# 011235813/discrete_mean_field_game

Hardware: AMD Instinct MI355X
Metric: env-steps/sec for batched d-bin population rollouts (higher is better)
Workload: dtype f32 (f64 accumulate); 1 GPU; actor_critic.train(update_every="rollout") of the drop-in class (mfg_ac2.train call surface; device-side start draw every episode, one update per 15-step rollout): d=21 topics, T=15, global batch 65536 = 65536 trajectories per GPU x 1; d=21, T=15, batch_per_gpu=65536, global_batch=65536, rng=philox4x32-10, parallelism=trajectory-sharded x1, 1 all-reduce/update

## Files before the change

### discrete_mean_field_game_amd/csrc/mfg_batch_sums.hip

```cpp
#include <hip/hip_runtime.h>
#include <limits.h>
#include <stdint.h>

#include "../../include/mfg_hip.h"
#include "mfg_batch_sums.h"
#include "mfg_core.h"
#include "mfg_grad.h"
#include "mfg_host.h"
#include "mfg_population.h"

using namespace mfg;

__global__ __launch_bounds__(BLOCK) void k_grad_partial(GradArgs a) { grad_partial_body(a); }

__global__ void k_add_reward(double* __restrict__ delta, const float* __restrict__ reward, int64_t N) {
  for (int64_t n = blockIdx.x * (int64_t)blockDim.x + threadIdx.x; n < N; n += (int64_t)gridDim.x * blockDim.x)
    delta[n] += (double)reward[n];
}

__global__ __launch_bounds__(RP_SLICES* RP_OUT) void k_reduce_partials(const double* __restrict__ partial, int64_t nsb, int64_t FO,
                                                                      int accumulate, double* __restrict__ G, ReduceApply ap) { reduce_partials_body(partial, nsb, FO, accumulate, G, ap); }

constexpr unsigned GM2_RECT44 = 0xFFFFu, GM2_DIAG44 = 0x8CEFu, GM2_DIAG44M = 0x0CEFu, GM2_TRAP24 = 0xEFu, GM2_RECT24 = 0xFFu,
                   GM2_ONE = 1u;
__host__ __device__ constexpr int gm2_count(unsigned m) { return m == 0 ? 0 : (int)(m & 1u) + gm2_count(m >> 1); }

template <int D, int NA, int NB, unsigned MASK>
__device__ __forceinline__ void gm2_step(const float* __restrict__ abase, const float* __restrict__ bbase, int off, double dk,
                                         v4d_t* acc) {
  double av[NA], bv[NB];
#pragma unroll
  for (int i = 0; i < NA; ++i) av[i] = dk * (double)abase[off + (i << 4)];
#pragma unroll
  for (int j = 0; j < NB; ++j) bv[j] = (double)bbase[off + (j << 4)];
  int t = 0;
#pragma unroll
  for (int i = 0; i < NA; ++i) {
#pragma unroll
    for (int j = 0; j < NB; ++j) {
      if ((MASK >> (i * NB + j)) & 1u) {
        acc[t] = __builtin_amdgcn_mfma_f64_16x16x4f64(av[i], bv[j], acc[t], 0, 0, 0);
        ++t;
      }
    }
  }
}
template <int D, int NA0, int NB0, unsigned M0, int NA1, int NB1, unsigned M1>
__device__ __forceinline__ void gm2_chunk(const float* __restrict__ sp, const double* __restrict__ dl, int lk, int li,
                                          const int* ra, const int* cb, v4d_t* acc) {
  constexpr int pitch = D + 16;
  const float* lb = sp + lk * pitch + li;
  const float *a0 = lb + (ra[0] << 4), *b0 = lb + (cb[0] << 4), *a1 = lb + (ra[1] << 4), *b1 = lb + (cb[1] << 4);
#pragma unroll 2
  for (int ks = 0; ks < GM_KC / 4; ++ks) {
    const double dk = dl[ks * 4 + lk];
    gm2_step<D, NA0, NB0, M0>(a0, b0, ks * 4 * pitch, dk, acc);
    if constexpr (M1 != 0) gm2_step<D, NA1, NB1, M1>(a1, b1, ks * 4 * pitch, dk, acc + gm2_count(M0));
  }
}
template <int D, int NA, int NB, unsigned MASK>
__device__ __forceinline__ void gm2_store(double* __restrict__ out, int lk, int li, int ra, int cb, const v4d_t* acc) {
  int t = 0;
#pragma unroll
  for (int i = 0; i < NA; ++i) {
#pragma unroll
    for (int j = 0; j < NB; ++j) {
      if ((MASK >> (i * NB + j)) & 1u) {
#pragma unroll
        for (int v = 0; v < 4; ++v) {
          const int gi = ((ra + i) << 4) + 4 * v + lk, gj = ((cb + j) << 4) + li;
          if (gi <= gj) out[feat_idx(gi, gj, D)] = acc[t][v];
        }
        ++t;
      }
    }
  }
}

template <int D>
struct Gm2Geom {
  static constexpr int NY = D == 256 ? 2 : 1, ACCN = D == 256 ? 17 : 9;
};
template <int NA_, int NB_, unsigned MASK_>
struct Gm2Rect {
  static constexpr int NA = NA_, NB = NB_;
  static constexpr unsigned MASK = MASK_;
};
template <int D>
__global__ __launch_bounds__(BLOCK, 2) void k_grad_mfma2(GradArgs a) {
  static_assert(D == 128 || D == 256, "tile maps exist for d = 128 and 256");
  extern __shared__ __attribute__((aligned(16))) unsigned char smem_raw[];
  constexpr int d = D, pitch = D + 16;
  constexpr int Q = d * (d + 1) / 2, F = Q + d + 1, FO = F + 3;
  constexpr int ACCN = Gm2Geom<D>::ACCN;
  double* dl = reinterpret_cast<double*>(smem_raw);
  double* red = dl + GM_KC;
  float* sp = reinterpret_cast<float*>(red + 4 * BLOCK);
  const int tid = threadIdx.x, lane = tid & (WAVE - 1);
  const int wv = __builtin_amdgcn_readfirstlane(tid / WAVE), y = (int)blockIdx.y;
  const bool diag = D == 256 ? wv == 3 : wv >= 2;
  int ra[2] = {0, 0}, cb[2] = {0, 0};
  if (D == 256) {
    const int sd = 2 * y;
    if (diag) {
      ra[0] = cb[0] = 4 * sd;
      ra[1] = cb[1] = 4 * sd + 4;
    } else {
      const int sr = y == 0 ? 0 : (wv == 2 ? 2 : 1), sc = y == 0 ? wv + 1 : (wv == 0 ? 2 : 3);
      ra[0] = 4 * sr;
      cb[0] = 4 * sc;
      ra[1] = 4 * sd + 4 + (wv == 2 ? 3 : 2);
      cb[1] = 4 * sd + 4 + (wv == 0 ? 2 : 3);
    }
  } else {
    if (diag) ra[0] = cb[0] = 4 * (wv - 2);
    else {
      ra[0] = 2 * wv;
      cb[0] = 4;
      ra[1] = cb[1] = 4 * wv + 3;
    }
  }
  const bool side = blockIdx.y == 0;
  double lin = 0.0, s_d = 0.0, s_dg = 0.0, s_r = 0.0, s_n = 0.0;
  const int li = lane & 15, lk = lane >> 4;
  const double invT = 1.0 / (double)a.T;
  constexpr int dq = d >> 2, rpp = BLOCK / dq, NPF = GM_KC / rpp;
  static_assert(BLOCK % dq == 0 && GM_KC % rpp == 0, "whole rows per staging pass");
  const int q0 = tid / dq, c4 = tid - q0 * dq;
  double* out = a.partial + (int64_t)blockIdx.x * FO;
  auto run = [&](auto r0, auto r1) __attribute__((always_inline)) {
    using R0 = decltype(r0);
    using R1 = decltype(r1);
    v4d_t acc[ACCN];
#pragma unroll
    for (int i = 0; i < ACCN; ++i) acc[i] = (v4d_t)(0.0);
    float4 pf[NPF];
    double pf_de = 0.0, pf_dg = 0.0, pf_rr = 0.0;
    bool pf_on = false;
    auto fetch = [&](int64_t n0_) __attribute__((always_inline)) {
      const int cn_ = (int)((a.N - n0_) < GM_KC ? (a.N - n0_) : GM_KC);
#pragma unroll
      for (int u = 0; u < NPF; ++u) {
        const int q = q0 + u * rpp;
        pf[u] = make_float4(0.f, 0.f, 0.f, 0.f);
        if (q < cn_) {
          const int64_t n = n0_ + q;
          const int64_t b = (int64_t)(((double)n + 0.5) * invT);
          pf[u] = *reinterpret_cast<const float4*>(a.pi + b * a.stride_b + (n - b * a.T) * d + 4 * c4);
        }
      }
      pf_de = 0.0, pf_dg = 0.0, pf_rr = 0.0, pf_on = false;
      if (tid < cn_) {
        const int64_t n = n0_ + tid;
        pf_de = a.delta[n];
        pf_rr = a.reward ? (double)a.reward[n] : 0.0;
// ... 145 lines not shown
  const double invT = 1.0 / (double)TP1;
  const int64_t npass = (N + VM2_MB - 1) / VM2_MB;
  const int ur = tid >> 2, uc = (tid & 3) << 4;
  const int xr = tid >> 4, xc = (tid & 15) << 2;
  double ustg[16];
  float4 xstg[8];
  for (int64_t pass = blockIdx.x; pass < npass; pass += gridDim.x) {
    const int64_t n0 = pass * VM2_MB;
    const float* xrow[8];
#pragma unroll
    for (int u = 0; u < 8; ++u) {
      int64_t n = n0 + xr + 16 * u;
      if (n >= N) n = N - 1;
      const int64_t b = (int64_t)(((double)n + 0.5) * invT);
      xrow[u] = pi + b * stride_b + (n - b * TP1) * (int64_t)d;
    }
    auto fetch = [&](int cbk, int kc) __attribute__((always_inline)) {
      const int k = VM2_KC * kc + ur, c0 = 64 * cbk + uc;
      const double* wr = w + ((int64_t)k * d - ((int64_t)k * (k - 1)) / 2 - k);
#pragma unroll
      for (int q = 0; q < 16; ++q) ustg[q] = (c0 + q >= k) ? wr[c0 + q] : 0.0;
#pragma unroll
      for (int u = 0; u < 8; ++u) xstg[u] = *reinterpret_cast<const float4*>(xrow[u] + VM2_KC * kc + xc);
    };
    auto commit = [&]() __attribute__((always_inline)) {
#pragma unroll
      for (int q = 0; q < 16; q += 2) *reinterpret_cast<double2*>(Us + ur * 64 + uc + q) = make_double2(ustg[q], ustg[q + 1]);
#pragma unroll
      for (int u = 0; u < 8; ++u) {
        float* dst = Xs + (xr + 16 * u) * VM2_XP + xc;
        *reinterpret_cast<float2*>(dst) = make_float2(xstg[u].x, xstg[u].y);
        *reinterpret_cast<float2*>(dst + 2) = make_float2(xstg[u].z, xstg[u].w);
      }
    };
    double vs[2][4] = {{0.0, 0.0, 0.0, 0.0}, {0.0, 0.0, 0.0, 0.0}};
    fetch(0, 0);
    for (int cbk = 0; cbk < ncb; ++cbk) {
      v4d_t acc[2][4];
#pragma unroll
      for (int sg = 0; sg < 2; ++sg)
#pragma unroll
        for (int cg = 0; cg < 4; ++cg) acc[sg][cg] = (v4d_t)(0.0);
      for (int kc = 0; kc <= cbk; ++kc) {
        __syncthreads();
        commit();
        __syncthreads();
        const bool last_kc = kc == cbk;
        if (!last_kc || cbk + 1 < ncb) fetch(last_kc ? cbk + 1 : cbk, last_kc ? 0 : kc + 1);
        const float* xa = Xs + (wv * 32 + li) * VM2_XP + lk;
        const double* ub = Us + lk * 64 + li;
        if (!last_kc) {
#pragma unroll 2
          for (int ks = 0; ks < VM2_KC / 4; ++ks) {
            const double a0 = (double)xa[4 * ks], a1 = (double)xa[16 * VM2_XP + 4 * ks];
#pragma unroll
            for (int cg = 0; cg < 4; ++cg) {
              const double bv = ub[4 * ks * 64 + 16 * cg];
              acc[0][cg] = __builtin_amdgcn_mfma_f64_16x16x4f64(a0, bv, acc[0][cg], 0, 0, 0);
              acc[1][cg] = __builtin_amdgcn_mfma_f64_16x16x4f64(a1, bv, acc[1][cg], 0, 0, 0);
            }
          }
        } else {
#pragma unroll
          for (int pq = 0; pq < 4; ++pq) {
#pragma unroll 2
            for (int ks = 4 * pq; ks < 4 * pq + 4; ++ks) {
              const double a0 = (double)xa[4 * ks], a1 = (double)xa[16 * VM2_XP + 4 * ks];
#pragma unroll
              for (int cg = pq; cg < 4; ++cg) {
                const double bv = ub[4 * ks * 64 + 16 * cg];
                acc[0][cg] = __builtin_amdgcn_mfma_f64_16x16x4f64(a0, bv, acc[0][cg], 0, 0, 0);
                acc[1][cg] = __builtin_amdgcn_mfma_f64_16x16x4f64(a1, bv, acc[1][cg], 0, 0, 0);
              }
            }
          }
        }
      }
#pragma unroll
      for (int cg = 0; cg < 4; ++cg) {
        const double bc = w[Q + 64 * cbk + 16 * cg + li];
#pragma unroll
        for (int sg = 0; sg < 2; ++sg) {
#pragma unroll
          for (int v = 0; v < 4; ++v) {
            const double x = (double)Xs[(wv * 32 + sg * 16 + 4 * v + lk) * VM2_XP + 16 * cg + li];
            vs[sg][v] = fma(acc[sg][cg][v] + bc, x, vs[sg][v]);
          }
        }
      }
    }
#pragma unroll
    for (int sg = 0; sg < 2; ++sg) {
#pragma unroll
      for (int v = 0; v < 4; ++v) {
        double t = vs[sg][v];
        t += dpp_mov_f64<0xB1, 0xF>(t);
        t += dpp_mov_f64<0x4E, 0xF>(t);
        t += dpp_mov_f64<0x141, 0xF>(t);
        t += dpp_mov_f64<0x140, 0xF>(t);
        const int64_t n = n0 + wv * 32 + sg * 16 + 4 * v + lk;
        if (li == 0 && n < N) V[n] = t + w[Q + d];
      }
    }
  }
}

__global__ void k_td_delta(const double* __restrict__ V, const float* __restrict__ reward, int64_t B, int T, double gamma,
                           int discount_pow, double* __restrict__ delta) {
  const int64_t n_tot = B * T;
  for (int64_t n = blockIdx.x * (int64_t)blockDim.x + threadIdx.x; n < n_tot; n += (int64_t)gridDim.x * blockDim.x) {
    const int64_t b = n / T;
    const int s = (int)(n - b * T);
    double gd = gamma;
    if (discount_pow) {
      gd = 1.0;
      for (int q = 0; q < s; ++q) gd *= gamma;
    }
    const double r = reward ? (double)reward[n] : 0.0;
    delta[n] = r + gd * V[b * (T + 1) + s + 1] - V[b * (T + 1) + s];
  }
}


namespace mfg {

bool value_batch_ok(int d) { return d > WAVE && d % 16 == 0 && d <= MFG_MAX_D; }
size_t value_buffer_bytes(int64_t N, int d) { return value_batch_ok(d) ? (size_t)(2 * N) * 8 : 0; }

void grad_geometry(int64_t N, int d, int* chunk, int64_t* nsb, int* nob) {
  const int64_t FO = mfg_num_features(d) + 3;
  int ch = 8192 / d;
  if (ch > 64) ch = 64;
  if (ch < 8) ch = 8;
  *chunk = ch;
  int64_t sb = (N + ch - 1) / ch;
#ifndef MFG_GRAD_WS_MB
#define MFG_GRAD_WS_MB 72
#endif
  int64_t cap = (int64_t)((long long)MFG_GRAD_WS_MB << 20) / (FO * 8);
  if (cap > 1024) cap = 1024;
  if (cap < 16) cap = 16;
  if (sb > cap) sb = cap;
  if (sb < 1) sb = 1;
  *nsb = sb;
  *nob = (int)((FO + GR_OUT_PER_BLOCK - 1) / GR_OUT_PER_BLOCK);
}

void launch_reduce_partials(const double* partial, int64_t nsb, int64_t FO, int accumulate, double* G, const ReduceApply& ap,
                            hipStream_t st) {
  hipLaunchKernelGGL(k_reduce_partials, dim3((unsigned)((FO + RP_OUT - 1) / RP_OUT)), dim3(RP_SLICES * RP_OUT), 0, st, partial, nsb,
                     FO, accumulate, G, ap);
}

int launch_grad(const float* pi, int64_t stride_b, const double* delta, const double* g, const float* reward, int64_t N, int T,
                int d, double* G, int accumulate, void* ws, size_t ws_bytes, hipStream_t st, const ApplyArgs* apply, bool* applied,
                bool add_reward, const PopArgs* pop) {
  if (applied) *applied = false;
  if (d <= MFG_GRAD_SMALL_MAX_D && T > INT_MAX - GS_CH)
    return fail(MFG_EUNSUPPORTED, "batch sums, d <= %d: T = %d above 2^31 - 65", MFG_GRAD_SMALL_MAX_D, T);
  const int64_t FO = mfg_num_features(d) + 3;
  int chunk, nob;
  int64_t nsb;
  grad_geometry(N, d, &chunk, &nsb, &nob);
  const size_t need = (size_t)(nsb * FO * 8) + MFG_WS_CONTROL_BYTES;
  if (ws_bytes < need) return fail(MFG_EWORKSPACE, "%s: need %lld bytes, have %lld", "workspace", (long long)need,
                                   (long long)ws_bytes);
  ReduceApply rap{};
  if (apply && !accumulate) {
    rap.on = 1;
    rap.lr_c = apply->lr_c;
    rap.lr_a = apply->lr_a;
    rap.count = (double)N;
    rap.w = apply->w;
    rap.theta = apply->theta;
    rap.reward_acc = apply->reward_acc;
  }
  GradArgs a{};
  a.pi = pi;
  a.stride_b = stride_b;
  a.delta = delta;
  a.g = g;
  a.reward = reward;
  a.N = N;
  a.T = T;
  a.d = d;
  a.chunk = chunk;
  a.nsb = nsb;
  a.partial = reinterpret_cast<double*>((char*)ws + MFG_WS_CONTROL_BYTES);
  const bool small = d <= MFG_GRAD_SMALL_MAX_D;
  if (add_reward && !small)
    hipLaunchKernelGGL(k_add_reward, dim3(grid_for(N, 256, 8)), dim3(256), 0, st, const_cast<double*>(delta), reward, N);
  if (small) {
    a.add_reward = add_reward ? 1 : 0;
    const int64_t NC = (N + GS_CH - 1) / GS_CH;
    int64_t blocks = (NC + WAVES - 1) / WAVES;
    const int64_t cap = (int64_t)num_cus() * MFG_GS_BPC;
    if (blocks > cap) blocks = cap;
    if (blocks > nsb) blocks = nsb;
    if (blocks < 1) blocks = 1;
    a.nsb = blocks;
    const bool fuse = blocks <= MFG_GRAD_FUSE_MAX_ROWS;
    if (fuse) {
      a.counter = reinterpret_cast<unsigned*>(ws);
      a.G = G;
      a.accumulate = accumulate;
      if (apply) {
        a.apply = 1;
        a.lr_c = apply->lr_c;
        a.lr_a = apply->lr_a;
        a.w = apply->w;
        a.theta = apply->theta;
        a.reward_acc = apply->reward_acc;
        if (applied) *applied = true;
      }
    }
    const bool wide = stride_b - (int64_t)T * d >= (1 << 23) || T >= MFG_GRAD_LONG_T;
    if (pop) {
      if (wide) return fail(MFG_EUNSUPPORTED, "%s", "population: trajectory stride or length beyond the small gradient kernel");
      launch_grad_mfma_small_pop(d == 21 || d == 15 ? d : 0, (unsigned)blocks, a, *pop, st);
      if (fuse) return check_launch("grad_mfma_small_pop");
      launch_reduce_partials_pop((unsigned)((FO + RP_OUT - 1) / RP_OUT), (const double*)a.partial, blocks, FO, G, rap, *pop, st);
      if (applied && rap.on) *applied = true;
      return check_launch("grad_mfma_small_pop");
    }
    if (wide) hipLaunchKernelGGL((k_grad_mfma_small<0, true>), dim3((unsigned)blocks), dim3(BLOCK), 0, st, a);
    else if (d == 21) hipLaunchKernelGGL((k_grad_mfma_small<21>), dim3((unsigned)blocks), dim3(BLOCK), 0, st, a);
    else if (d == 15) hipLaunchKernelGGL((k_grad_mfma_small<15>), dim3((unsigned)blocks), dim3(BLOCK), 0, st, a);
    else hipLaunchKernelGGL((k_grad_mfma_small<0>), dim3((unsigned)blocks), dim3(BLOCK), 0, st, a);
    if (fuse) return check_launch("grad_mfma_small");
    launch_reduce_partials(a.partial, blocks, FO, accumulate, G, rap, st);
    if (applied && rap.on) *applied = true;
    return check_launch("grad_mfma_small");
  }
  if (d % 16 == 0 && d >= 64 && d <= 4 * BLOCK) {
    const int nt = d / 16, ntiles = nt * (nt + 1) / 2;
    const int ny = (ntiles + WAVES * GM_TPW - 1) / (WAVES * GM_TPW);
    const int tpw = (ntiles + ny * WAVES - 1) / (ny * WAVES);
    a.chunk = (BLOCK % (d / 4) == 0 && (((uintptr_t)pi & 15) == 0) && (stride_b % 4 == 0)) ? 1 : 0;
    const size_t lds_m = (size_t)GM_KC * 8 + (size_t)4 * BLOCK * 8 + (size_t)GM_KC * (d + 16) * 4;
    const int npf = a.chunk ? d / 32 : 0;
    if (pop) {
      if (npf != 0 && npf != 2) return fail(MFG_EUNSUPPORTED, "%s", "population: d > 64");
      launch_grad_mfma_pop(npf, (unsigned)nsb, (unsigned)ny, lds_m, a, tpw, *pop, st);
      launch_reduce_partials_pop((unsigned)((FO + RP_OUT - 1) / RP_OUT), (const double*)a.partial, nsb, FO, G, rap, *pop, st);
      if (applied && rap.on) *applied = true;
      return check_launch("grad_mfma_pop");
    }
#ifndef MFG_GRAD_MFMA_OLD
    if (a.chunk && (d == 128 || d == 256)) {
#ifndef MFG_GM2_BPC128
#define MFG_GM2_BPC128 3
#endif
      const int64_t want = d == 256 ? (int64_t)num_cus() * 2 / Gm2Geom<256>::NY : (int64_t)num_cus() * MFG_GM2_BPC128 / Gm2Geom<128>::NY;
      if (nsb > want) nsb = want;
      a.nsb = nsb;
      if (d == 256) hipLaunchKernelGGL((k_grad_mfma2<256>), dim3((unsigned)nsb, (unsigned)Gm2Geom<256>::NY), dim3(BLOCK), lds_m, st, a);
      else hipLaunchKernelGGL((k_grad_mfma2<128>), dim3((unsigned)nsb, (unsigned)Gm2Geom<128>::NY), dim3(BLOCK), lds_m, st, a);
    } else
#endif
    switch (npf) {
      case 2: hipLaunchKernelGGL((k_grad_mfma<2>), dim3((unsigned)nsb, (unsigned)ny), dim3(BLOCK), lds_m, st, a, tpw); break;
      case 4: hipLaunchKernelGGL((k_grad_mfma<4>), dim3((unsigned)nsb, (unsigned)ny), dim3(BLOCK), lds_m, st, a, tpw); break;
      case 8: hipLaunchKernelGGL((k_grad_mfma<8>), dim3((unsigned)nsb, (unsigned)ny), dim3(BLOCK), lds_m, st, a, tpw); break;
      case 16: hipLaunchKernelGGL((k_grad_mfma<16>), dim3((unsigned)nsb, (unsigned)ny), dim3(BLOCK), lds_m, st, a, tpw); break;
      default: hipLaunchKernelGGL((k_grad_mfma<0>), dim3((unsigned)nsb, (unsigned)ny), dim3(BLOCK), lds_m, st, a, tpw); break;
    }
    launch_reduce_partials(a.partial, nsb, FO, accumulate, G, rap, st);
    if (applied && rap.on) *applied = true;
    return check_launch("grad_mfma");
  }
  const size_t lds = (size_t)chunk * 3 * 8 + (size_t)chunk * d * 4;
  if (pop) {
    launch_grad_partial_pop((unsigned)nsb, (unsigned)nob, lds, a, *pop, st);
    launch_reduce_partials_pop((unsigned)((FO + RP_OUT - 1) / RP_OUT), (const double*)a.partial, nsb, FO, G, rap, *pop, st);
    if (applied && rap.on) *applied = true;
    return check_launch("grad_partial_pop");
  }
  hipLaunchKernelGGL(k_grad_partial, dim3((unsigned)nsb, (unsigned)nob), dim3(BLOCK), lds, st, a);
  launch_reduce_partials(a.partial, nsb, FO, accumulate, G, rap, st);
  if (applied && rap.on) *applied = true;
  return check_launch("grad_reduce");
}

int launch_values_and_delta(const float* pi_traj, int64_t B, int T, int d, const double* w, const float* reward,
                                   double gamma, int discount_pow, double* delta, void* ws, size_t ws_bytes, hipStream_t st) {
  const int64_t N = B * T, NV = B * (int64_t)(T + 1);
  int chunk, nob;
  int64_t nsb;
  grad_geometry(N, d, &chunk, &nsb, &nob);
  const size_t off = (size_t)(nsb * (mfg_num_features(d) + 3) * 8) + MFG_WS_CONTROL_BYTES;
  if (!ws || ws_bytes < off + (size_t)NV * 8)
    return fail(MFG_EWORKSPACE, "%s: need %lld bytes, have %lld", "values", (long long)(off + (size_t)NV * 8), (long long)ws_bytes);
  double* V = reinterpret_cast<double*>((char*)ws + off);
  const size_t lds = (size_t)WAVES * 16 * (d + 4) * 4 + (size_t)2 * VM_CH * 16 * 8;
  int64_t groups = (NV + 15) / 16;
  int64_t blocks = (groups + WAVES - 1) / WAVES;
  const int64_t cap = (int64_t)num_cus() * 8;
  if (blocks > cap) blocks = cap;
#ifndef MFG_VALUE_MFMA_OLD
  if (d % 64 == 0) {
    const size_t lds2 = (size_t)VM2_KC * 64 * 8 + (size_t)VM2_MB * VM2_XP * 4;
    int64_t blocks2 = (NV + VM2_MB - 1) / VM2_MB;
    if (blocks2 > (int64_t)num_cus() * 2) blocks2 = (int64_t)num_cus() * 2;
    hipLaunchKernelGGL(k_value_mfma2, dim3((unsigned)blocks2), dim3(BLOCK), lds2, st, pi_traj, (int64_t)(T + 1) * d, NV, T + 1, d, w, V);
  } else
#endif
  hipLaunchKernelGGL(k_value_mfma, dim3((unsigned)blocks), dim3(BLOCK), lds, st, pi_traj, (int64_t)(T + 1) * d, NV, T + 1, d, w, V);
  hipLaunchKernelGGL(k_td_delta, dim3(grid_for(N, 256, 8)), dim3(256), 0, st, (const double*)V, reward, B, T, gamma, discount_pow,
                     delta);
  return check_launch("values");
}

}
```

### discrete_mean_field_game_amd/csrc/mfg_grad.h

```cpp
#pragma once
#include <hip/hip_runtime.h>
#include <stdint.h>

#include "mfg_core.h"

using namespace mfg;

constexpr int MFG_GRAD_SMALL_MAX_D = 28;
constexpr int GR_OUT_PER_THREAD = 4;
constexpr int GR_OUT_PER_BLOCK = GR_OUT_PER_THREAD * BLOCK;

struct GradArgs {
  const float* pi;
  int64_t stride_b;
  const double* delta;
  const double* g;
  const float* reward;
  int64_t N;
  int T, d, chunk;
  int64_t nsb;
  double* partial;
  int add_reward;
  unsigned* counter;
  double* G;
  int accumulate, apply;
  double lr_c, lr_a;
  double *w, *theta, *reward_acc;
};

__device__ __forceinline__ void grad_partial_body(const GradArgs& a) {
  extern __shared__ __attribute__((aligned(16))) unsigned char smem_raw[];
  const int d = a.d, Q = d * (d + 1) / 2, F = Q + d + 1, FO = F + 3;
  double* dl = reinterpret_cast<double*>(smem_raw);
  float* sp = reinterpret_cast<float*>(dl + 3 * a.chunk);
  const int tid = threadIdx.x;
  int oi[GR_OUT_PER_THREAD], oj[GR_OUT_PER_THREAD], kind[GR_OUT_PER_THREAD];
  double acc[GR_OUT_PER_THREAD];
#pragma unroll
  for (int u = 0; u < GR_OUT_PER_THREAD; ++u) {
    const int k = blockIdx.y * GR_OUT_PER_BLOCK + u * BLOCK + tid;
    acc[u] = 0.0;
    oi[u] = oj[u] = 0;
    if (k < Q) {
      int i = (int)(((2.0 * d + 1.0) - sqrt((2.0 * d + 1.0) * (2.0 * d + 1.0) - 8.0 * (double)k)) * 0.5);
      while (i > 0 && feat_idx(i, i, d) > k) --i;
      while (i + 1 < d && feat_idx(i + 1, i + 1, d) <= k) ++i;
      oi[u] = i;
      oj[u] = i + (k - feat_idx(i, i, d));
      kind[u] = 0;
    } else if (k < Q + d) {
      oi[u] = k - Q;
      kind[u] = 1;
    } else if (k < FO) {
      kind[u] = 2 + (k - (Q + d));
    } else {
      kind[u] = -1;
    }
  }
  for (int64_t n0 = (int64_t)blockIdx.x * a.chunk; n0 < a.N; n0 += a.nsb * a.chunk) {
    const int cn = (int)((a.N - n0) < a.chunk ? (a.N - n0) : a.chunk);
    __syncthreads();
    for (int k = tid; k < cn * d; k += BLOCK) {
      const int q = k / d, c = k - q * d;
      const int64_t n = n0 + q;
      const int64_t b = n / a.T;
      const int s = (int)(n - b * a.T);
      sp[k] = a.pi[b * a.stride_b + (int64_t)s * d + c];
    }
    for (int q = tid; q < cn; q += BLOCK) {
      const double de = a.delta[n0 + q];
      dl[3 * q] = de;
      dl[3 * q + 1] = a.g ? de * a.g[n0 + q] : 0.0;
      dl[3 * q + 2] = a.reward ? (double)a.reward[n0 + q] : 0.0;
    }
    __syncthreads();
#pragma unroll
    for (int u = 0; u < GR_OUT_PER_THREAD; ++u) {
      double s_ = acc[u];
      if (kind[u] == 0) {
        for (int q = 0; q < cn; ++q) s_ = fma(dl[3 * q] * (double)sp[q * d + oi[u]], (double)sp[q * d + oj[u]], s_);
      } else if (kind[u] == 1) {
        for (int q = 0; q < cn; ++q) s_ = fma(dl[3 * q], (double)sp[q * d + oi[u]], s_);
      } else if (kind[u] == 2) {
        for (int q = 0; q < cn; ++q) s_ += dl[3 * q];
      } else if (kind[u] == 3) {
        for (int q = 0; q < cn; ++q) s_ += dl[3 * q + 1];
      } else if (kind[u] == 4) {
        for (int q = 0; q < cn; ++q) s_ += dl[3 * q + 2];
      } else if (kind[u] == 5) {
        s_ += (double)cn;
      }
      acc[u] = s_;
    }
  }
#pragma unroll
  for (int u = 0; u < GR_OUT_PER_THREAD; ++u) {
    const int k = blockIdx.y * GR_OUT_PER_BLOCK + u * BLOCK + tid;
    if (kind[u] >= 0) a.partial[(int64_t)blockIdx.x * FO + k] = acc[u];
  }
}

constexpr int GS_CH = 64;
#ifndef MFG_GS_BPC
#define MFG_GS_BPC 2
#endif

template <int D>
struct GradChunk {
  static constexpr int NL = D ? D : MFG_GRAD_SMALL_MAX_D;
  float pi[NL];
  double de, dg;
  float rr;
};

constexpr int MFG_GRAD_LONG_T = 1 << 22;
__device__ __forceinline__ int grad_boundaries_wide(int sj, int T, float invT) {
  return T >= GS_CH ? (int)(sj >= T) : (int)(((float)sj + 0.5f) * invT);
}
template <int D, bool WIDE>
__device__ __forceinline__ void grad_chunk_load(GradChunk<D>& c, const GradArgs& a, const double* gp, const float* rp, int d,
                                                int64_t n0, int64_t b0, int s0, int lane, float invT, float inv_d) {
  const int last = (int)((a.N - 1 - n0) < (GS_CH - 1) ? (a.N - 1 - n0) : (GS_CH - 1));
  {
    const int64_t n = n0 + (lane < last ? lane : last);
    c.de = a.delta[n];
    c.dg = gp[n];
    c.rr = rp[n];
  }
  if constexpr (!WIDE) {
    const float* cb = a.pi + b0 * a.stride_b + (int64_t)s0 * d;
    const int extra = (int)(a.stride_b - (int64_t)a.T * d);
#pragma unroll
    for (int k = 0; k < GradChunk<D>::NL; ++k) {
      if (!D && k * WAVE >= GS_CH * d) {
        c.pi[k] = 0.0f;
        continue;
      }
      int e = k * WAVE + lane;
      int j = (int)(((float)e + 0.5f) * inv_d);
      if (j > last) { j = last; e = last * d; }
      const int q = (int)(((float)(s0 + j) + 0.5f) * invT);
      c.pi[k] = cb[(unsigned)(e + __mul24(q, extra))];
    }
  } else {
#pragma unroll
    for (int k = 0; k < GradChunk<D>::NL; ++k) {
      if (!D && k * WAVE >= GS_CH * d) {
        c.pi[k] = 0.0f;
        continue;
      }
      const int e = k * WAVE + lane;
      int j = (int)(((float)e + 0.5f) * inv_d);
      int col = e - j * d;
      if (j > last) { j = last; col = 0; }
      const int sj = s0 + j;
      const int q = grad_boundaries_wide(sj, a.T, invT);
      const int64_t off = (b0 + q) * a.stride_b + ((int64_t)(sj - q * a.T) * d + col);
      c.pi[k] = a.pi[off];
    }
  }
}

template <int D, bool WIDE>
__device__ __forceinline__ void grad_mfma_small_body(const GradArgs& a) {
  const int d = D ? D : a.d;
  const int Q = d * (d + 1) / 2, F = Q + d + 1, FO = F + 3;
  constexpr int DMAX = D ? D : MFG_GRAD_SMALL_MAX_D;
  constexpr int PI_FL = GS_CH * DMAX + 16;
  constexpr int W_BYTES = ((PI_FL * 4 + 15) / 16) * 16 + GS_CH * 3 * 8;
  constexpr int RED_BYTES = WAVES * 3 * 4 * WAVE * 8;
  __shared__ __attribute__((aligned(16))) unsigned char smem[(WAVES * W_BYTES > RED_BYTES) ? WAVES * W_BYTES : RED_BYTES];
  const int tid = threadIdx.x, lane = tid & (WAVE - 1), wv = __builtin_amdgcn_readfirstlane(tid / WAVE);
  float* lpi = reinterpret_cast<float*>(smem + (size_t)wv * W_BYTES);
  double* lsc = reinterpret_cast<double*>(smem + (size_t)wv * W_BYTES + ((PI_FL * 4 + 15) / 16) * 16);
  const int li = lane & 15, lk = lane >> 4;
  auto consts = [&](int idx, float& a_d, double& a_1, float& b_1, double& b_g, double& b_r) {
    a_d = idx == d ? 1.0f : 0.0f;
    a_1 = idx == d + 1 ? 1.0 : 0.0;
    b_1 = (idx == d || idx == d + 3) ? 1.0f : 0.0f;
    b_g = idx == d + 1 ? 1.0 : 0.0;
    b_r = idx == d + 2 ? 1.0 : 0.0;
  };
  float ad_lo, b1_lo, ad_hi, b1_hi;
  double a1_lo, a1_hi, bg_lo, br_lo, bg_hi, br_hi;
  consts(li, ad_lo, a1_lo, b1_lo, bg_lo, br_lo);
  consts(16 + li, ad_hi, a1_hi, b1_hi, bg_hi, br_hi);
  const bool pi_lo = li < d, pi_hi = 16 + li < d;
  const int ilo = pi_lo ? li : 0, ihi = pi_hi ? 16 + li : 0;
  const bool has_g = a.g != nullptr, has_r = a.reward != nullptr;
  const double* gp = has_g ? a.g : a.delta;
  const float* rp = has_r ? a.reward : a.pi;
  v4d_t c00 = (v4d_t)(0.0), c01 = (v4d_t)(0.0), c11 = (v4d_t)(0.0);
  const float invT = 1.0f / (float)a.T, inv_d = 1.0f / (float)d;
  const int64_t NC = (a.N + GS_CH - 1) / GS_CH;
  const int64_t W = (int64_t)gridDim.x * WAVES;
  const int64_t gw = (int64_t)blockIdx.x * WAVES + wv;
  GradChunk<D> nx;
  if (gw < NC) grad_chunk_load<D, WIDE>(nx, a, gp, rp, d, gw * GS_CH, (gw * GS_CH) / a.T, (int)((gw * GS_CH) % a.T), lane, invT, inv_d);
  for (int64_t ch = gw; ch < NC; ch += W) {
    const int64_t n0 = ch * GS_CH;
    __builtin_amdgcn_s_waitcnt(0xc07f);
    __builtin_amdgcn_wave_barrier();
#pragma unroll
    for (int k = 0; k < GradChunk<D>::NL; ++k)
      if (D || k * WAVE < GS_CH * d) lpi[k * WAVE + lane] = nx.pi[k];
    {
      const bool ok = n0 + lane < a.N;
      const double rr = (ok && has_r) ? (double)nx.rr : 0.0;
      double de = ok ? nx.de : 0.0;
      if (a.add_reward) {
        de += rr;
        if (ok) const_cast<double*>(a.delta)[n0 + lane] = de;
      }
      lsc[3 * lane] = de;
      lsc[3 * lane + 1] = (ok && has_g) ? nx.dg : 0.0;
      lsc[3 * lane + 2] = rr;
    }
    const int nvalid = (int)((a.N - n0) < GS_CH ? (a.N - n0) : GS_CH);
    if (ch + W < NC) {
      const int64_t n1 = (ch + W) * GS_CH;
      grad_chunk_load<D, WIDE>(nx, a, gp, rp, d, n1, n1 / a.T, (int)(n1 % a.T), lane, invT, inv_d);
    }
    __builtin_amdgcn_s_waitcnt(0xc07f);
    __builtin_amdgcn_wave_barrier();
#pragma unroll 4
    for (int ks = 0; ks < GS_CH / 4; ++ks) {
      const int j = 4 * ks + lk;
      const float plo = lpi[j * d + ilo], phi = lpi[j * d + ihi];
      const double de = lsc[3 * j], dg = lsc[3 * j + 1];
      const double rr = lsc[3 * j + 2];
      const double one = j < nvalid ? 1.0 : 0.0;
      double A_lo, B_lo;
      if constexpr (D >= 16) {
        B_lo = (double)plo;
        A_lo = de * B_lo;
      } else {
        A_lo = fma(de, (double)(pi_lo ? plo : ad_lo), a1_lo * one);
        B_lo = fma(bg_lo, dg, fma(br_lo, rr, (double)(pi_lo ? plo : b1_lo)));
      }
      const double A_hi = fma(de, (double)(pi_hi ? phi : ad_hi), a1_hi * one);
      const double B_hi = fma(bg_hi, dg, fma(br_hi, rr, (double)(pi_hi ? phi : b1_hi)));
      c00 = __builtin_amdgcn_mfma_f64_16x16x4f64(A_lo, B_lo, c00, 0, 0, 0);
      c01 = __builtin_amdgcn_mfma_f64_16x16x4f64(A_lo, B_hi, c01, 0, 0, 0);
      c11 = __builtin_amdgcn_mfma_f64_16x16x4f64(A_hi, B_hi, c11, 0, 0, 0);
    }
  }
  __syncthreads();
  double (*red)[3][4][WAVE] = reinterpret_cast<double (*)[3][4][WAVE]>(smem);
#pragma unroll
  for (int v = 0; v < 4; ++v) {
    red[wv][0][v][lane] = c00[v];
    red[wv][1][v][lane] = c01[v];
    red[wv][2][v][lane] = c11[v];
  }
  __syncthreads();
  double* out = a.partial + (int64_t)blockIdx.x * FO;
  for (int e = tid; e < 3 * 4 * WAVE; e += BLOCK) {
    const int t = e / (4 * WAVE), v = (e / WAVE) & 3, l = e & (WAVE - 1);
    const int gi = (t == 2 ? 16 : 0) + 4 * v + (l >> 4), gj = (t == 0 ? 0 : 16) + (l & 15);
    int k = -1;
    if (gj < d) {
      if (gi <= gj) k = feat_idx(gi, gj, d);
    } else if (gj == d) {
      if (gi <= d) k = Q + gi;
    } else if (gj == d + 1) {
      if (gi == d) k = F;
    } else if (gj == d + 2) {
      if (gi == d + 1) k = F + 1;
    } else if (gj == d + 3) {
      if (gi == d + 1) k = F + 2;
    }
    if (k >= 0) {
      double tsum = red[0][t][v][l];
#pragma unroll
      for (int q = 1; q < WAVES; ++q) tsum += red[q][t][v][l];
      out[k] = tsum;
    }
  }
  if (!a.counter) return;
  __shared__ int s_last;
  __threadfence();
  __syncthreads();
  if (tid == 0) s_last = (atomicAdd(a.counter, 1u) == gridDim.x - 1) ? 1 : 0;
  __syncthreads();
  if (!s_last) return;
  __threadfence();
  double* fin = &red[0][0][0][0];
  const int nrows = (int)gridDim.x;
  for (int k = tid; k < FO; k += BLOCK) {
    double s0 = 0.0, s1 = 0.0, s2 = 0.0, s3 = 0.0;
    const double* col = a.partial + k;
    int r = 0;
    for (; r + 7 < nrows; r += 8) {
      const double v0 = col[(int64_t)r * FO], v1 = col[(int64_t)(r + 1) * FO], v2 = col[(int64_t)(r + 2) * FO],
                   v3 = col[(int64_t)(r + 3) * FO], v4 = col[(int64_t)(r + 4) * FO], v5 = col[(int64_t)(r + 5) * FO],
                   v6 = col[(int64_t)(r + 6) * FO], v7 = col[(int64_t)(r + 7) * FO];
      s0 += v0;
      s1 += v1;
      s2 += v2;
      s3 += v3;
      s0 += v4;
      s1 += v5;
      s2 += v6;
      s3 += v7;
    }
    for (; r < nrows; ++r) s0 += col[(int64_t)r * FO];
    const double tot = (s0 + s1) + (s2 + s3);
    const double gk = a.accumulate ? a.G[k] + tot : tot;
    a.G[k] = gk;
    fin[k] = gk;
  }
  __syncthreads();
  if (a.apply) {
    const double count = fin[F + 2];
    if (count > 0.0) {
      const double inv = 1.0 / count;
      for (int k = tid; k < F; k += BLOCK) a.w[k] = updated_param(a.w[k], a.lr_c, fin[k], inv);
      if (tid == 0) {
        if (a.reward_acc) *a.reward_acc += fin[F + 1] * inv;
        *a.theta = updated_param(*a.theta, a.lr_a, fin[F], inv);
      }
    }
  }
  if (tid == 0) *a.counter = 0u;
}
template <int D, bool WIDE = false>
__global__ __launch_bounds__(BLOCK) void k_grad_mfma_small(GradArgs a) { grad_mfma_small_body<D, WIDE>(a); }

constexpr int GM_KC = 32;
#ifndef MFG_GM_TPW
#define MFG_GM_TPW 8
#endif
constexpr int GM_TPW = MFG_GM_TPW;

template <int NPF>
__device__ __forceinline__ void grad_mfma_body(const GradArgs& a, int tpw) {
  extern __shared__ __attribute__((aligned(16))) unsigned char smem_raw[];
  const int d = a.d, nt = d >> 4, pitch = d + 16;
  const int Q = d * (d + 1) / 2, F = Q + d + 1, FO = F + 3;
  double* dl = reinterpret_cast<double*>(smem_raw);
  double* red = dl + GM_KC;
  float* sp = reinterpret_cast<float*>(red + 4 * BLOCK);
  const int tid = threadIdx.x, lane = tid & (WAVE - 1), wv = tid / WAVE;
  const int ntiles = nt * (nt + 1) / 2;
  const int t0 = ((int)blockIdx.y * WAVES + wv) * tpw;
  int nmine = ntiles - t0;
  nmine = nmine < 0 ? 0 : (nmine > tpw ? tpw : nmine);
  int tr[GM_TPW], tc[GM_TPW];
#pragma unroll
  for (int i = 0; i < GM_TPW; ++i) {
    int t = t0 + i, r = 0;
    if (i < nmine) {
      while (t >= nt - r) {
        t -= nt - r;
        ++r;
      }
    } else {
      t = 0;
    }
    tr[i] = r;
    tc[i] = r + t;
  }
  v4d_t acc[GM_TPW];
#pragma unroll
  for (int i = 0; i < GM_TPW; ++i) acc[i] = (v4d_t)(0.0);
  const bool side = blockIdx.y == 0;
  double lin[4] = {0.0, 0.0, 0.0, 0.0}, s_d = 0.0, s_dg = 0.0, s_r = 0.0, s_n = 0.0;
  const int li = lane & 15, lk = lane >> 4;
  const double invT = 1.0 / (double)a.T;
  const int dq = d >> 2, rpp = BLOCK / (dq > 0 ? dq : 1);
  const int q0 = tid / dq, c4 = tid - q0 * dq;
  float4 pf[NPF > 0 ? NPF : 1];
  double pf_de = 0.0, pf_dg = 0.0, pf_rr = 0.0;
  bool pf_on = false;
#define MFG_GM_FETCH(n0_)                                                                              \
  {                                                                                                    \
    const int cn_ = (int)((a.N - (n0_)) < GM_KC ? (a.N - (n0_)) : GM_KC);                              \
    _Pragma("unroll") for (int u = 0; u < NPF; ++u) {                                                  \
      const int q = q0 + u * rpp;                                                                      \
      pf[u] = make_float4(0.f, 0.f, 0.f, 0.f);                                                         \
      if (q < cn_) {                                                                                   \
        const int64_t n = (n0_) + q;                                                                   \
        const int64_t b = (int64_t)(((double)n + 0.5) * invT);                                         \
        pf[u] = *reinterpret_cast<const float4*>(a.pi + b * a.stride_b + (n - b * a.T) * d + 4 * c4);  \
      }                                                                                                \
    }                                                                                                  \
    pf_de = 0.0; pf_dg = 0.0; pf_rr = 0.0; pf_on = false;                                              \
    if (tid < cn_) {                                                                                   \
      const int64_t n = (n0_) + tid;                                                                   \
      pf_de = a.delta[n];                                                                              \
      pf_rr = a.reward ? (double)a.reward[n] : 0.0;                                                    \
      if (a.g) pf_dg = a.g[n];                                                                         \
      pf_on = true;                                                                                    \
    }                                                                                                  \
  }
  if (NPF > 0 && (int64_t)blockIdx.x * GM_KC < a.N) MFG_GM_FETCH((int64_t)blockIdx.x * GM_KC)
  for (int64_t n0 = (int64_t)blockIdx.x * GM_KC; n0 < a.N; n0 += (int64_t)gridDim.x * GM_KC) {
    const int cn = (int)((a.N - n0) < GM_KC ? (a.N - n0) : GM_KC);
    __syncthreads();
// ... 190 lines not shown
```

Measured before the change: 1.104 billion env-steps/s.

## Restructure small-d gradient loop with padded LDS rows and buffer loads

Replaces the inner loop of the small-d MFMA gradient kernel with a version that stores each chunk row in a padded LDS layout holding pi values plus per-row scalars (delta, g, reward, live, one, zero). Operand selection then becomes precomputed byte offsets instead of per-iteration selects and FMAs. Full chunks are fetched with raw buffer loads using incrementally advanced trajectory/step indices rather than per-element divisions. It also grows the LDS footprint, and the old loop stays reachable through an environment variable.

```diff
diff --git a/discrete_mean_field_game_amd/csrc/mfg_batch_sums.hip b/discrete_mean_field_game_amd/csrc/mfg_batch_sums.hip
--- a/discrete_mean_field_game_amd/csrc/mfg_batch_sums.hip
+++ b/discrete_mean_field_game_amd/csrc/mfg_batch_sums.hip
@@ -1,6 +1,8 @@
 #include <hip/hip_runtime.h>
 #include <limits.h>
 #include <stdint.h>
+#include <stdlib.h>
+#include <string.h>
 
 #include "../../include/mfg_hip.h"
 #include "mfg_batch_sums.h"
@@ -452,6 +454,11 @@
                      FO, accumulate, G, ap);
 }
 
+static int grad_ref_loop_asked() {
+  const char* e = getenv("MFG_GRAD_BODY");
+  return (e && !strcmp(e, "ref")) ? 1 : 0;
+}
+
 int launch_grad(const float* pi, int64_t stride_b, const double* delta, const double* g, const float* reward, int64_t N, int T,
                 int d, double* G, int accumulate, void* ws, size_t ws_bytes, hipStream_t st, const ApplyArgs* apply, bool* applied,
                 bool add_reward, const PopArgs* pop) {
@@ -492,6 +499,7 @@
     hipLaunchKernelGGL(k_add_reward, dim3(grid_for(N, 256, 8)), dim3(256), 0, st, const_cast<double*>(delta), reward, N);
   if (small) {
     a.add_reward = add_reward ? 1 : 0;
+    a.ref_loop = grad_ref_loop_asked();
     const int64_t NC = (N + GS_CH - 1) / GS_CH;
     int64_t blocks = (NC + WAVES - 1) / WAVES;
     const int64_t cap = (int64_t)num_cus() * MFG_GS_BPC;
diff --git a/discrete_mean_field_game_amd/csrc/mfg_grad.h b/discrete_mean_field_game_amd/csrc/mfg_grad.h
--- a/discrete_mean_field_game_amd/csrc/mfg_grad.h
+++ b/discrete_mean_field_game_amd/csrc/mfg_grad.h
@@ -26,6 +26,7 @@
   int accumulate, apply;
   double lr_c, lr_a;
   double *w, *theta, *reward_acc;
+  int ref_loop;
 };
 
 __device__ __forceinline__ void grad_partial_body(const GradArgs& a) {
@@ -161,18 +162,19 @@
   }
 }
 
+template <int D>
+struct GradSmallRefLds {
+  static constexpr int DMAX = D ? D : MFG_GRAD_SMALL_MAX_D;
+  static constexpr int PI_FL = GS_CH * DMAX + 16;
+  static constexpr int PI_BYTES = ((PI_FL * 4 + 15) / 16) * 16;
+  static constexpr int W_BYTES = PI_BYTES + GS_CH * 3 * 8;
+};
 template <int D, bool WIDE>
-__device__ __forceinline__ void grad_mfma_small_body(const GradArgs& a) {
-  const int d = D ? D : a.d;
-  const int Q = d * (d + 1) / 2, F = Q + d + 1, FO = F + 3;
-  constexpr int DMAX = D ? D : MFG_GRAD_SMALL_MAX_D;
-  constexpr int PI_FL = GS_CH * DMAX + 16;
-  constexpr int W_BYTES = ((PI_FL * 4 + 15) / 16) * 16 + GS_CH * 3 * 8;
-  constexpr int RED_BYTES = WAVES * 3 * 4 * WAVE * 8;
-  __shared__ __attribute__((aligned(16))) unsigned char smem[(WAVES * W_BYTES > RED_BYTES) ? WAVES * W_BYTES : RED_BYTES];
-  const int tid = threadIdx.x, lane = tid & (WAVE - 1), wv = __builtin_amdgcn_readfirstlane(tid / WAVE);
+__device__ __forceinline__ void grad_small_loop_ref(const GradArgs& a, unsigned char* smem, int d, int lane, int wv, v4d_t& c00,
+                                                    v4d_t& c01, v4d_t& c11) {
+  constexpr int W_BYTES = GradSmallRefLds<D>::W_BYTES;
   float* lpi = reinterpret_cast<float*>(smem + (size_t)wv * W_BYTES);
-  double* lsc = reinterpret_cast<double*>(smem + (size_t)wv * W_BYTES + ((PI_FL * 4 + 15) / 16) * 16);
+  double* lsc = reinterpret_cast<double*>(smem + (size_t)wv * W_BYTES + GradSmallRefLds<D>::PI_BYTES);
   const int li = lane & 15, lk = lane >> 4;
   auto consts = [&](int idx, float& a_d, double& a_1, float& b_1, double& b_g, double& b_r) {
     a_d = idx == d ? 1.0f : 0.0f;
@@ -190,7 +192,6 @@
   const bool has_g = a.g != nullptr, has_r = a.reward != nullptr;
   const double* gp = has_g ? a.g : a.delta;
   const float* rp = has_r ? a.reward : a.pi;
-  v4d_t c00 = (v4d_t)(0.0), c01 = (v4d_t)(0.0), c11 = (v4d_t)(0.0);
   const float invT = 1.0f / (float)a.T, inv_d = 1.0f / (float)d;
   const int64_t NC = (a.N + GS_CH - 1) / GS_CH;
   const int64_t W = (int64_t)gridDim.x * WAVES;
@@ -245,6 +246,164 @@
       c11 = __builtin_amdgcn_mfma_f64_16x16x4f64(A_hi, B_hi, c11, 0, 0, 0);
     }
   }
+}
+
+template <int D>
+struct GradSmallRow {
+  static constexpr int DMAX = D ? D : MFG_GRAD_SMALL_MAX_D;
+  static constexpr int ZF = DMAX * 4;
+  static constexpr int SC = ((DMAX + 1) * 4 + 7) / 8 * 8;
+  static constexpr int O_DE = SC, O_G = SC + 8, O_R = SC + 16, O_LIVE = SC + 24, O_ONE = SC + 32, O_ZERO = SC + 40;
+  static constexpr int RP = SC + 48;
+  static constexpr int W_BYTES = GS_CH * RP;
+};
+
+__device__ __forceinline__ int64_t grad_wave_uniform(int64_t v) {
+  const unsigned lo = (unsigned)__builtin_amdgcn_readfirstlane((int)v), hi = (unsigned)__builtin_amdgcn_readfirstlane((int)(v >> 32));
+  return (int64_t)(((uint64_t)hi << 32) | lo);
+}
+
+template <int D>
+__device__ __forceinline__ void grad_chunk_load_full(GradChunk<D>& c, const GradArgs& a, const double* gp, const float* rp, int d,
+                                                     int64_t n0, int64_t b0, int s0, int lane, float invT,
+                                                     const float (&fj)[GradChunk<D>::NL]) {
+  {
+    const int64_t n = n0 + lane;
+    c.de = a.delta[n];
+    c.dg = gp[n];
+    c.rr = rp[n];
+  }
+  const float* cb = reinterpret_cast<const float*>(grad_wave_uniform((int64_t)(a.pi + b0 * a.stride_b + (int64_t)s0 * d)));
+  const int extra = (int)(a.stride_b - (int64_t)a.T * d);
+  const __amdgpu_buffer_rsrc_t rs = __builtin_amdgcn_make_buffer_rsrc(const_cast<float*>(cb), 0, -1, 0x00020000);
+  const float fs0 = (float)s0;
+#pragma unroll
+  for (int k = 0; k < GradChunk<D>::NL; ++k) {
+    if (!D && k * WAVE >= GS_CH * d) {
+      c.pi[k] = 0.0f;
+      continue;
+    }
+    const int off4 = 4 * __mul24((int)((fj[k] + fs0) * invT), extra);
+    c.pi[k] = __builtin_bit_cast(float, __builtin_amdgcn_raw_buffer_load_b32(rs, 4 * lane + off4, k * WAVE * 4, 0));
+  }
+}
+
+template <int D, bool WIDE>
+__device__ __forceinline__ void grad_small_loop(const GradArgs& a, unsigned char* smem, int d, int lane, int wv, v4d_t& c00,
+                                                v4d_t& c01, v4d_t& c11) {
+  using R = GradSmallRow<D>;
+  unsigned char* wb = smem + (size_t)wv * R::W_BYTES;
+  const int li = lane & 15, lk = lane >> 4;
+  auto sources = [&](int idx, int& o_pi, int& o_a, int& o_b) {
+    o_pi = idx < d ? idx * 4 : R::ZF;
+    o_a = idx == d ? R::O_DE : idx == d + 1 ? R::O_LIVE : R::O_ZERO;
+    o_b = (idx == d || idx == d + 3) ? R::O_ONE : idx == d + 1 ? R::O_G : idx == d + 2 ? R::O_R : R::O_ZERO;
+  };
+  int pi_lo, a_lo, b_lo, pi_hi, a_hi, b_hi;
+  sources(li, pi_lo, a_lo, b_lo);
+  sources(16 + li, pi_hi, a_hi, b_hi);
+  const unsigned char* r0 = wb + lk * R::RP;
+  const bool has_g = a.g != nullptr, has_r = a.reward != nullptr;
+  const double* gp = has_g ? a.g : a.delta;
+  const float* rp = has_r ? a.reward : a.pi;
+  const float invT = 1.0f / (float)a.T, inv_d = 1.0f / (float)d;
+  const int64_t NC = (a.N + GS_CH - 1) / GS_CH;
+  const int64_t W = (int64_t)gridDim.x * WAVES;
+  const int64_t gw = (int64_t)blockIdx.x * WAVES + wv;
+  if (gw >= NC) return;
+  int jk4[GradChunk<D>::NL];
+  float fj[GradChunk<D>::NL];
+#pragma unroll
+  for (int k = 0; k < GradChunk<D>::NL; ++k) {
+    const int j = (int)(((float)(k * WAVE + lane) + 0.5f) * inv_d);
+    jk4[k] = 4 * j;
+    fj[k] = (float)j + 0.5f;
+  }
+  const int row_gap4 = R::RP / 4 - d;
+  {
+    unsigned char* row = wb + lane * R::RP;
+    *reinterpret_cast<float*>(row + R::ZF) = 0.0f;
+    *reinterpret_cast<double*>(row + R::O_ONE) = 1.0;
+    *reinterpret_cast<double*>(row + R::O_ZERO) = 0.0;
+  }
+  const int64_t stride_n = W * GS_CH, stride_tr = grad_wave_uniform(stride_n / a.T), stride_st = grad_wave_uniform(stride_n % a.T);
+  int64_t n0 = gw * GS_CH, b0 = grad_wave_uniform(n0 / a.T), s0 = grad_wave_uniform(n0 % a.T);
+  GradChunk<D> nx;
+  auto load = [&](int64_t n, int64_t b, int64_t s) {
+    if constexpr (!WIDE) {
+      if (a.N - n >= GS_CH) {
+        grad_chunk_load_full<D>(nx, a, gp, rp, d, n, b, (int)s, lane, invT, fj);
+        return;
+      }
+    }
+    grad_chunk_load<D, WIDE>(nx, a, gp, rp, d, n, b, (int)s, lane, invT, inv_d);
+  };
+  load(n0, b0, s0);
+  for (int64_t ch = gw; ch < NC; ch += W) {
+    __builtin_amdgcn_s_waitcnt(0xc07f);
+    __builtin_amdgcn_wave_barrier();
+#pragma unroll
+    for (int k = 0; k < GradChunk<D>::NL; ++k)
+      if (D || k * WAVE < GS_CH * d)
+        *reinterpret_cast<float*>(wb + 4 * (k * WAVE + lane) + jk4[k] * row_gap4) = nx.pi[k];
+    {
+      const bool ok = n0 + lane < a.N;
+      const double rr = (ok && has_r) ? (double)nx.rr : 0.0;
+      double de = ok ? nx.de : 0.0;
+      if (a.add_reward) {
+        de += rr;
+        if (ok) const_cast<double*>(a.delta)[n0 + lane] = de;
+      }
+      unsigned char* row = wb + lane * R::RP;
+      *reinterpret_cast<double*>(row + R::O_DE) = de;
+      *reinterpret_cast<double*>(row + R::O_G) = (ok && has_g) ? nx.dg : 0.0;
+      *reinterpret_cast<double*>(row + R::O_R) = rr;
+      *reinterpret_cast<double*>(row + R::O_LIVE) = ok ? 1.0 : 0.0;
+    }
+    n0 += stride_n;
+    b0 += stride_tr;
+    s0 += stride_st;
+    if (s0 >= a.T) {
+      s0 -= a.T;
+      ++b0;
+    }
+    if (ch + W < NC) load(n0, b0, s0);
+    __builtin_amdgcn_s_waitcnt(0xc07f);
+    __builtin_amdgcn_wave_barrier();
+#pragma unroll 4
+    for (int ks = 0; ks < GS_CH / 4; ++ks) {
+      const unsigned char* r = r0 + ks * 4 * R::RP;
+      const double xlo = (double)*reinterpret_cast<const float*>(r + pi_lo);
+      const double xhi = (double)*reinterpret_cast<const float*>(r + pi_hi);
+      const double de = *reinterpret_cast<const double*>(r + R::O_DE);
+      double A_lo, B_lo;
+      if constexpr (D >= 16) {
+        B_lo = xlo;
+        A_lo = de * B_lo;
+      } else {
+        A_lo = fma(de, xlo, *reinterpret_cast<const double*>(r + a_lo));
+        B_lo = xlo + *reinterpret_cast<const double*>(r + b_lo);
+      }
+      const double A_hi = fma(de, xhi, *reinterpret_cast<const double*>(r + a_hi));
+      const double B_hi = xhi + *reinterpret_cast<const double*>(r + b_hi);
+      c00 = __builtin_amdgcn_mfma_f64_16x16x4f64(A_lo, B_lo, c00, 0, 0, 0);
+      c01 = __builtin_amdgcn_mfma_f64_16x16x4f64(A_lo, B_hi, c01, 0, 0, 0);
+      c11 = __builtin_amdgcn_mfma_f64_16x16x4f64(A_hi, B_hi, c11, 0, 0, 0);
+    }
+  }
+}
+
+template <int D, bool WIDE>
+__device__ __forceinline__ void grad_mfma_small_body(const GradArgs& a) {
+  const int d = D ? D : a.d;
+  const int Q = d * (d + 1) / 2, F = Q + d + 1, FO = F + 3;
+  constexpr int W_BYTES = GradSmallRow<D>::W_BYTES > GradSmallRefLds<D>::W_BYTES ? GradSmallRow<D>::W_BYTES : GradSmallRefLds<D>::W_BYTES;
+  constexpr int RED_BYTES = WAVES * 3 * 4 * WAVE * 8;
+  __shared__ __attribute__((aligned(16))) unsigned char smem[(WAVES * W_BYTES > RED_BYTES) ? WAVES * W_BYTES : RED_BYTES];
+  const int tid = threadIdx.x, lane = tid & (WAVE - 1), wv = __builtin_amdgcn_readfirstlane(tid / WAVE);
+  v4d_t c00 = (v4d_t)(0.0), c01 = (v4d_t)(0.0), c11 = (v4d_t)(0.0);
+  if (a.ref_loop) grad_small_loop_ref<D, WIDE>(a, smem, d, lane, wv, c00, c01, c11);
+  else grad_small_loop<D, WIDE>(a, smem, d, lane, wv, c00, c01, c11);
   __syncthreads();
   double (*red)[3][4][WAVE] = reinterpret_cast<double (*)[3][4][WAVE]>(smem);
 #pragma unroll
```

After: 1.111 billion env-steps/s (median of 6 runs). No clear change (+0.7%).
